# mparker97/deflate_compression

Measured on AMD Instinct MI355X. Metric: encode GB/s (uncompressed in) + compression ratio vs CPU ref, 1/2/4/8 MI355X, higher is better.
Workload: dtype u8; 1 GPU; C3: enwik8-sized enwik-style wiki text (seeded generator); bytes_per_rank=100000000, block=32768, parse=max_chain=7, lazy, store-check, deep, parallelism=blocks sharded over 1 GPU(s)

## Files before the change

deflate_compression_amd/csrc/dmx_kernels.hip:

```cpp
#include <hip/hip_runtime.h>
#include <stdint.h>
#include <stdio.h>
#include <stdlib.h>
#include <string.h>

#include "dmx_internal.h"
#include "../../include/dmx.h"

#define MAXLEN 258


__device__ __forceinline__ uint32_t dmx_hash(uint32_t tri) { return (tri * 0x9E3779B1u) >> DMX_HASH_SHIFT; }
__device__ __forceinline__ uint32_t wave_of(uint32_t tid) { return (uint32_t)__builtin_amdgcn_readfirstlane((int)(tid >> 6)); }
__device__ __forceinline__ uint32_t sort_key(uint32_t w, uint32_t p) { return (dmx_hash(w & 0xFFFFFFu) << 15) | p; }
__device__ __forceinline__ uint32_t dmx_hash4(uint32_t w) { return (w * 0x9E3779B1u) >> DMX_HASH_SHIFT; }
template <int NB>
__device__ __forceinline__ uint32_t bucket_of(uint64_t w) {
    if (NB == 3) return dmx_hash((uint32_t)w & 0xFFFFFFu);
    if (NB == 4) return dmx_hash4((uint32_t)w);
    return (uint32_t)(((w & 0xFFFFFFFFFFull) * 0x9E3779B97F4A7C15ull) >> (64 - 13));
}
template <int NB>
__device__ __forceinline__ uint32_t sort_key_h(uint64_t w, uint32_t p) { return (bucket_of<NB>(w) << 15) | p; }
template <int NB>
// ... 14 lines not shown
__device__ __forceinline__ void dist_sym(uint32_t dist, uint32_t& sym, uint32_t& eb, uint32_t& ev) {
    uint32_t x = dist - 1;
    if (x < 4) { sym = x; eb = 0; ev = 0; }
    else {
        uint32_t e = 31 - __clz(x);
        eb = e - 1;
        sym = 2 * e + ((x >> (e - 1)) & 1);
        ev = x & ((1u << eb) - 1);
    }
}

__device__ __forceinline__ uint32_t len_eb_of_sym(uint32_t s) {
    return (s >= 265 && s < 285) ? (s - 261) / 4 : 0;
}
__device__ __forceinline__ uint32_t dist_eb_of_sym(uint32_t s) { return s < 4 ? 0 : s / 2 - 1; }
__device__ __forceinline__ uint32_t fixed_len(uint32_t s) { return s < 144 ? 8 : s < 256 ? 9 : s < 280 ? 7 : 8; }

#define DMX_DPP_SHR(x, n) ((uint32_t)__builtin_amdgcn_update_dpp(0, (int)(x), 0x110 + (n), 0xF, 0xF, true))
__device__ __forceinline__ uint32_t wave_sum_u32(uint32_t v) {
    v += DMX_DPP_SHR(v, 1);
    v += DMX_DPP_SHR(v, 2);
    v += DMX_DPP_SHR(v, 4);
    v += DMX_DPP_SHR(v, 8);
    return __builtin_amdgcn_readlane(v, 15) + __builtin_amdgcn_readlane(v, 31) + __builtin_amdgcn_readlane(v, 47) +
           __builtin_amdgcn_readlane(v, 63);
}
__device__ __forceinline__ uint64_t dpp_shr64(uint64_t v, int n) {
    const uint32_t lo = (uint32_t)v, hi = (uint32_t)(v >> 32);
    uint32_t a, b;
    switch (n) {
        case 1: a = DMX_DPP_SHR(lo, 1); b = DMX_DPP_SHR(hi, 1); break;
        case 2: a = DMX_DPP_SHR(lo, 2); b = DMX_DPP_SHR(hi, 2); break;
        case 4: a = DMX_DPP_SHR(lo, 4); b = DMX_DPP_SHR(hi, 4); break;
        default: a = DMX_DPP_SHR(lo, 8); b = DMX_DPP_SHR(hi, 8); break;
    }
    return (uint64_t)a | ((uint64_t)b << 32);
}
__device__ __forceinline__ uint64_t readlane64(uint64_t v, int l) {
    return (uint64_t)(uint32_t)__builtin_amdgcn_readlane((int)(uint32_t)v, l) |
           ((uint64_t)(uint32_t)__builtin_amdgcn_readlane((int)(uint32_t)(v >> 32), l) << 32);
}
__device__ __forceinline__ uint32_t wave_claim(uint32_t* ctr) {
#ifdef DMX_CHECK_CLAIM
    if (__builtin_amdgcn_read_exec() != ~0ull) __builtin_trap();
#endif
    return atomicAdd(ctr, 1u) >> 6;
}
__device__ __forceinline__ uint64_t wave_sum_u64(uint64_t v) {
    v += dpp_shr64(v, 1);
    v += dpp_shr64(v, 2);
    v += dpp_shr64(v, 4);
    v += dpp_shr64(v, 8);
    return readlane64(v, 15) + readlane64(v, 31) + readlane64(v, 47) + readlane64(v, 63);
}


#define MT 1024
#define MW (MT / 64)
#define DMX_STAMPS 16
#define DATA_WORDS 8272

struct __attribute__((aligned(16))) MatchLDS {
    uint32_t data[DATA_WORDS];
    uint16_t sorted[DMX_BLK];
    uint16_t bstart[DMX_NBUCKET];
    uint8_t len8[DMX_BLK];
    uint32_t lit[DMX_BLK / 32];
    uint32_t tsm[DMX_BLK / 32];
    uint32_t exitp[DMX_BLK / 32];
    uint32_t hist[DMX_HIST];
    uint32_t wexit[MW];
    uint32_t wsum[MW];
    uint32_t ntok;
    uint32_t sortbad;
    unsigned long long adl_s, adl_t;
};

__device__ __forceinline__ uint64_t fsh64(uint64_t lo, uint64_t hi, uint32_t sh) {
    return sh ? ((lo >> sh) | (hi << (64 - sh))) : lo;
}
__device__ __forceinline__ uint64_t ld8(const uint32_t* W, uint32_t p) {
    const uint32_t a = p >> 2, sh = p & 3;
    const uint32_t w0 = W[a], w1 = W[a + 1], w2 = W[a + 2];
    return (uint64_t)__builtin_amdgcn_alignbyte(w1, w0, sh) | ((uint64_t)__builtin_amdgcn_alignbyte(w2, w1, sh) << 32);
}
__device__ __forceinline__ uint32_t ld4(const uint32_t* W, uint32_t p) {
    return __builtin_amdgcn_alignbyte(W[(p >> 2) + 1], W[p >> 2], p & 3);
}
template <int NB>
__device__ __forceinline__ uint64_t ldg(const uint32_t* W, uint32_t p) { return NB > 4 ? ld8(W, p) : (uint64_t)ld4(W, p); }
template <int NG>
__device__ __forceinline__ uint16_t seed_enc(uint32_t q) {
    return q != 0xFFFFu ? (uint16_t)((NG == 4 ? 0x8000u : 0u) | q) : (uint16_t)0xFFFFu;
}
__device__ __forceinline__ uint32_t seed_dec(uint32_t s) {
    return s == 0xFFFFu ? 0u : ((3u + (s >> 15)) << 15) | (s & 0x7FFFu);
}
__device__ __forceinline__ void ld12(const uint32_t* W, uint32_t p, uint32_t& x0, uint32_t& x1, uint32_t& x2) {
    const uint32_t a = p >> 2, sh = p & 3;
    const uint32_t w0 = W[a], w1 = W[a + 1], w2 = W[a + 2], w3 = W[a + 3];
    x0 = __builtin_amdgcn_alignbyte(w1, w0, sh);
    x1 = __builtin_amdgcn_alignbyte(w2, w1, sh);
    x2 = __builtin_amdgcn_alignbyte(w3, w2, sh);
}

__device__ __forceinline__ uint32_t adv_of(const MatchLDS& L, uint32_t p) {
// ... 944 lines not shown
    if (__ballot(valid && v != v0) == 0) {
        if ((threadIdx.x & 63) == first) {
            const uint32_t c = (uint32_t)__popcll(vm);
            if (pair16) atomicAdd(&T[v0 >> 1], c << (16 * (v0 & 1)));
            else atomicAdd(&T[v0], c);
        }
    } else if (valid) {
        if (pair16) atomicAdd(&T[v >> 1], 1u << (16 * (v & 1)));
        else atomicAdd(&T[v], 1u);
    }
}

template <bool RUNCHK = true>
__device__ __forceinline__ uint32_t atomic_rank(uint32_t* T, uint32_t v, bool valid, uint64_t lt) {
    if (!RUNCHK) return valid ? atomicAdd(&T[v], 1u) : 0u;
    const uint64_t vm = __ballot(valid);
    if (vm == 0) return 0;
    const uint32_t first = (uint32_t)__builtin_ctzll(vm);
    const uint32_t v0 = __builtin_amdgcn_readlane(v, (int)first);
    if (__ballot(valid && v != v0) == 0) {
        uint32_t base = 0;
        if ((threadIdx.x & 63) == first) base = atomicAdd(&T[v0], (uint32_t)__popcll(vm));
        return __builtin_amdgcn_readlane(base, (int)first) + (uint32_t)__popcll(vm & lt);
    }
    return valid ? atomicAdd(&T[v], 1u) : 0u;
}

__device__ __forceinline__ uint32_t block_excl_scan(MatchLDS& L, uint32_t v, uint32_t tid) {
    const uint32_t incl = wave_incl_scan(v);
    if ((tid & 63) == 63) L.wsum[tid >> 6] = incl;
    __syncthreads();
    uint32_t base = 0;
    for (uint32_t w = 0; w < (tid >> 6); w++) base += L.wsum[w];
    __syncthreads();
    return base + incl - v;
}

template <bool RUNCHK>
__device__ __forceinline__ uint32_t atomic_rank16(uint32_t* T, uint32_t v, bool valid, uint64_t lt, uint32_t sh) {
    if (RUNCHK) {
        const uint64_t vm = __ballot(valid);
        if (vm == 0) return 0;
        const uint32_t first = (uint32_t)__builtin_ctzll(vm);
        const uint32_t v0 = __builtin_amdgcn_readlane(v, (int)first);
        if (__ballot(valid && v != v0) == 0) {
            uint32_t base = 0;
            if ((threadIdx.x & 63) == first) base = atomicAdd(&T[v0], (uint32_t)__popcll(vm) << sh);
            return ((__builtin_amdgcn_readlane(base, (int)first) >> sh) & 0xFFFFu) + (uint32_t)__popcll(vm & lt);
        }
    }
    return (atomicAdd(&T[v], valid ? 1u << sh : 0u) >> sh) & 0xFFFFu;
}

template <bool RUNCHK, int NB>
__device__ __forceinline__ void count_sort_positions(MatchLDS& L, uint32_t bn, int32_t max_chain, uint32_t tid,
                                                     bool stamp, uint64_t* tp0) {
    const uint32_t lane = tid & 63, wave = wave_of(tid);
    const uint32_t nvalid = bn > 2 ? bn - 2 : 0;
    const bool need_starts = max_chain <= 0 || max_chain > KD;
    uint32_t* T = reinterpret_cast<uint32_t*>(L.len8);
    const uint4 z4 = make_uint4(0, 0, 0, 0);
    reinterpret_cast<uint4*>(T)[tid] = z4;
    reinterpret_cast<uint4*>(T)[tid + MT] = z4;
    uint32_t* T2 = reinterpret_cast<uint32_t*>(L.sorted);
    reinterpret_cast<uint4*>(T2)[tid] = z4;
    reinterpret_cast<uint4*>(T2)[tid + MT] = z4;
    constexpr uint32_t NR = 4;
    uint32_t* Tg = (wave >> 3) ? T2 : T;
    const uint32_t sh = ((wave >> 2) & 1) << 4;
    __syncthreads();
    const uint64_t lt = (1ull << lane) - 1ull;
    uint32_t x0l = (wave << 11) + lane, nvl = nvalid;
    uint32_t hh[16];
    asm volatile("" : "+v"(x0l), "+v"(nvl));
#pragma unroll
    for (int st = 0; st < 32; st += 2) {
        const uint32_t xa = x0l + ((uint32_t)st << 6), xb = xa + 64;
        const uint32_t ha = xa < nvl ? bucket_of<NB>(ldg<NB>(L.data, xa)) : 0u;
        const uint32_t hb = xb < nvl ? bucket_of<NB>(ldg<NB>(L.data, xb)) : 0u;
        hh[st >> 1] = ha | (hb << 16);
        if ((st & 7) == 6) __builtin_amdgcn_sched_barrier(0);
    }
    if (stamp && tid == 0) tp0[0] = __builtin_amdgcn_s_memtime();
    uint32_t rk[16];
#pragma unroll
    for (int j = 0; j < 16; j++) rk[j] = 0;
    for (uint32_t r = 0; r < NR; r++) {
        if (r == (wave & (NR - 1))) {
            asm volatile("" : "+v"(x0l), "+v"(nvl));
            if (RUNCHK) {
#pragma unroll
                for (int st = 0; st < 32; st++) {
                    const uint32_t x = x0l + ((uint32_t)st << 6);
                    const uint32_t h = (hh[st >> 1] >> (16 * (st & 1))) & 0xFFFFu;
                    const uint32_t rr = atomic_rank16<true>(Tg, h, x < nvl, lt, sh);
                    rk[st >> 1] |= rr << (16 * (st & 1));
                }
            } else {
#pragma unroll
                for (int hb = 0; hb < 32; hb += 16) {
                    uint32_t old[16];
#pragma unroll
                    for (int q = 0; q < 16; q++) {
                        const int st = hb + q;
                        const uint32_t x = x0l + ((uint32_t)st << 6);
                        const uint32_t h = (hh[st >> 1] >> (16 * (st & 1))) & 0xFFFFu;
                        old[q] = atomicAdd(&Tg[h], x < nvl ? 1u << sh : 0u);
                    }
#pragma unroll
                    for (int q = 0; q < 16; q++) {
                        const int st = hb + q;
                        rk[st >> 1] |= ((old[q] >> sh) & 0xFFFFu) << (16 * (st & 1));
                    }
                }
            }
        }
        __syncthreads();
    }
    if (stamp && tid == 0) tp0[1] = __builtin_amdgcn_s_memtime();
    {
        const uint4 a = reinterpret_cast<const uint4*>(T)[2 * tid], c = reinterpret_cast<const uint4*>(T)[2 * tid + 1];
        uint32_t w[8] = {a.x, a.y, a.z, a.w, c.x, c.y, c.z, c.w}, pre[8], s = 0;
        const uint4 a2 = reinterpret_cast<const uint4*>(T2)[2 * tid], c2 = reinterpret_cast<const uint4*>(T2)[2 * tid + 1];
        uint32_t w2[8] = {a2.x, a2.y, a2.z, a2.w, c2.x, c2.y, c2.z, c2.w};
#pragma unroll
        for (int j = 0; j < 8; j++) {
            pre[j] = s;
            s += (w[j] & 0xFFFFu) + (w[j] >> 16);
            s += (w2[j] & 0xFFFFu) + (w2[j] >> 16);
        }
        const uint32_t base = block_excl_scan(L, s, tid);
#pragma unroll
        for (int j = 0; j < 8; j++) {
            const uint32_t st0 = base + pre[j];
            pre[j] = st0;
            const uint32_t s1 = st0 + (w[j] & 0xFFFFu), s2 = s1 + (w[j] >> 16);
            w[j] = st0 | (s1 << 16);
            w2[j] = s2 | ((s2 + (w2[j] & 0xFFFFu)) << 16);
        }
        reinterpret_cast<uint4*>(T)[2 * tid] = make_uint4(w[0], w[1], w[2], w[3]);
        reinterpret_cast<uint4*>(T)[2 * tid + 1] = make_uint4(w[4], w[5], w[6], w[7]);
        reinterpret_cast<uint4*>(T2)[2 * tid] = make_uint4(w2[0], w2[1], w2[2], w2[3]);
        reinterpret_cast<uint4*>(T2)[2 * tid + 1] = make_uint4(w2[4], w2[5], w2[6], w2[7]);
        if (need_starts)
            reinterpret_cast<uint4*>(L.bstart)[tid] = make_uint4(pre[0] | (pre[1] << 16), pre[2] | (pre[3] << 16),
                                                                 pre[4] | (pre[5] << 16), pre[6] | (pre[7] << 16));
    }
    __syncthreads();
    asm volatile("" : "+v"(x0l), "+v"(nvl));
#pragma unroll
    for (int st = 0; st < 32; st++) {
        const uint32_t h = (hh[st >> 1] >> (16 * (st & 1))) & 0xFFFFu;
        const uint32_t rr = (rk[st >> 1] >> (16 * (st & 1))) & 0xFFFFu;
        const uint32_t dst = ((Tg[h] >> sh) & 0xFFFFu) + rr;
        rk[st >> 1] = (rk[st >> 1] & (0xFFFF0000u >> (16 * (st & 1)))) | ((dst & 0xFFFFu) << (16 * (st & 1)));
        if ((st & 7) == 7) __builtin_amdgcn_sched_barrier(0);
    }
    __syncthreads();
#pragma unroll
    for (int st = 0; st < 32; st++) {
        const uint32_t x = x0l + ((uint32_t)st << 6);
        if (x < nvl) L.sorted[(rk[st >> 1] >> (16 * (st & 1))) & 0xFFFFu] = (uint16_t)x;
    }
    __syncthreads();
    if (stamp && tid == 0) tp0[2] = __builtin_amdgcn_s_memtime();
}

template <bool EXACT, bool RUNCHK = true, int NB = 3>
__device__ __forceinline__ void sort_positions(MatchLDS& L, uint32_t bn, int32_t max_chain, uint32_t tid, bool stamp,
                                               uint64_t* tp0) {
    if constexpr (!EXACT) {
        count_sort_positions<RUNCHK, NB>(L, bn, max_chain, tid, stamp, tp0);
        return;
    }
    const uint32_t lane = tid & 63, wave = wave_of(tid);
    const uint32_t nvalid = bn > 2 ? bn - 2 : 0;
    const bool need_starts = max_chain <= 0 || max_chain > KD;
    uint32_t* C = L.tsm;
    uint32_t* C2 = L.lit;
    uint8_t* D2 = reinterpret_cast<uint8_t*>(L.bstart);
    unsigned long long* G = reinterpret_cast<unsigned long long*>(L.len8 + DMX_BLK / 2);
    unsigned long long* Gw = G + (wave << 7);
    for (uint32_t k = tid; k < 2 * (DMX_BLK / 32); k += MT) C[k] = 0;
    for (uint32_t k = tid; k < DMX_BLK / 32; k += MT) C2[k] = 0;
    for (uint32_t k = tid; k < 16 * 128; k += MT) G[k] = 0;
    __syncthreads();
    if (stamp && tid == 0) tp0[0] = __builtin_amdgcn_s_memtime();
    const uint64_t lt = (1ull << lane) - 1ull;
    const uint32_t x0 = (wave << 11) + lane;
    uint32_t x0l = x0, nvl = nvalid;
    uint32_t hh[16];
    asm volatile("" : "+v"(x0l), "+v"(nvl));
#pragma unroll
    for (int st = 0; st < 32; st += 2) {
        const uint32_t xa = x0l + ((uint32_t)st << 6), xb = xa + 64;
        const uint32_t ha = xa < nvl ? bucket_of<NB>(ldg<NB>(L.data, xa)) : 0u;
        const uint32_t hb = xb < nvl ? bucket_of<NB>(ldg<NB>(L.data, xb)) : 0u;
        hh[st >> 1] = ha | (hb << 16);
        if ((st & 7) == 6) __builtin_amdgcn_sched_barrier(0);
    }
    asm volatile("" : "+v"(x0l), "+v"(nvl));
#pragma unroll
    for (int st = 0; st < 32; st++) {
        const uint32_t x = x0l + ((uint32_t)st << 6);
        const uint32_t h = (hh[st >> 1] >> (16 * (st & 1))) & 0xFFFFu;
        count_add<RUNCHK>(C + (wave << 7), h & 127u, x < nvl, false);
    }
    __syncthreads();
    {
        const uint32_t o0 = tid * 2, o1 = o0 + 1;
        const uint32_t i0 = ((o0 & 15) << 7) + (o0 >> 4), i1 = ((o1 & 15) << 7) + (o1 >> 4);
        const uint32_t v0 = C[i0], v1 = C[i1];
        const uint32_t ex = block_excl_scan(L, v0 + v1, tid);
        C[i0] = ex;
        C[i1] = ex + v0;
    }
    __syncthreads();
    asm volatile("" : "+v"(x0l), "+v"(nvl));
#pragma unroll
    for (int st = 0; st < 32; st++) {
        const uint32_t x = x0l + ((uint32_t)st << 6);
        const bool valid = x < nvl;
        const uint32_t h = (hh[st >> 1] >> (16 * (st & 1))) & 0xFFFFu;
        const uint32_t dg = h & 127u;
        uint32_t dst = 0;
        if (EXACT) {
            const uint32_t c = valid ? C[(wave << 7) + dg] : 0u;
// ... 14 lines not shown
    if (stamp && tid == 0) tp0[1] = __builtin_amdgcn_s_memtime();
    uint32_t pk[16], dk[8];
    asm volatile("" : "+v"(x0l), "+v"(nvl));
#pragma unroll
    for (int st = 0; st < 32; st += 2) {
        const uint32_t xa = x0l + ((uint32_t)st << 6), xb = xa + 64;
        const uint32_t pa = xa < nvl ? (uint32_t)L.sorted[xa] : 0u;
        const uint32_t pb = xb < nvl ? (uint32_t)L.sorted[xb] : 0u;
        const uint32_t da = xa < nvl ? (uint32_t)D2[xa] : 0u;
        const uint32_t db = xb < nvl ? (uint32_t)D2[xb] : 0u;
        pk[st >> 1] = pa | (pb << 16);
        if ((st & 3) == 0) dk[st >> 2] = da | (db << 8);
        else dk[st >> 2] |= (da << 16) | (db << 24);
        if ((st & 7) == 6) __builtin_amdgcn_sched_barrier(0);
    }
    {
        const uint32_t i0 = ((tid & 15) << 6) + (tid >> 4);
        const uint32_t v0 = C2[i0];
        const uint32_t ex = block_excl_scan(L, v0, tid);
        C2[i0] = ex;
    }
    __syncthreads();
    asm volatile("" : "+v"(x0l), "+v"(nvl));
#pragma unroll
    for (int st = 0; st < 32; st++) {
        const uint32_t x = x0l + ((uint32_t)st << 6);
        const bool valid = x < nvl;
        const uint32_t p = (pk[st >> 1] >> (16 * (st & 1))) & 0xFFFFu;
        const uint32_t dg = (dk[st >> 2] >> (8 * (st & 3))) & 0xFFu;
        if (EXACT) {
            const uint32_t c = valid ? C2[(wave << 6) + dg] : 0u;
            const uint64_t eq = group_of(Gw, dg, valid);
            if (valid) {
                L.sorted[c + (uint32_t)__popcll(eq & lt)] = (uint16_t)p;
                if ((eq >> lane) == 1ull) C2[(wave << 6) + dg] = c + (uint32_t)__popcll(eq);
            }
        } else {
            const uint32_t dst = atomic_rank<RUNCHK>(&C2[wave << 6], dg, valid, lt);
            if (valid) L.sorted[dst] = (uint16_t)p;
        }
        __builtin_amdgcn_sched_barrier(0);
    }
    __syncthreads();
    for (uint32_t k = tid; k < DMX_BLK / 32; k += MT) L.lit[k] = 0;
    if (need_starts) {
        for (uint32_t k = tid; k < nvalid; k += MT) {
            const uint32_t h = bucket_of<NB>(ldg<NB>(L.data, L.sorted[k]));
            const uint32_t hp = k ? bucket_of<NB>(ldg<NB>(L.data, L.sorted[k - 1])) : 0xFFFFFFFFu;
            if (h != hp) L.bstart[h] = (uint16_t)k;
        }
    }
    __syncthreads();
    if (stamp && tid == 0) tp0[2] = __builtin_amdgcn_s_memtime();
}


template <int NG>
__device__ __forceinline__ uint32_t gram_pass(MatchLDS& L, uint32_t nv, uint32_t tid, uint16_t* __restrict__ seeds,
                                              uint32_t& ndefer, uint64_t& tsweep) {
    constexpr uint32_t PW = 9;
    constexpr uint32_t GM = NG == 3 ? 0xFFFFFFu : 0xFFFFFFFFu;
    const uint32_t lane = tid & 63;
    uint32_t* UL = L.tsm;
    uint32_t bad = 0;
    if (tid == 0) { L.ntok = 0; L.wsum[0] = 0; L.wsum[1] = 0; }
    __syncthreads();
    uint32_t cnx = wave_claim(&L.wsum[0]);
    for (;;) {
        const uint32_t kb = (uint32_t)__builtin_amdgcn_readfirstlane((int)cnx) << 6;
        if (kb >= nv) break;
        cnx = wave_claim(&L.wsum[0]);
        const uint32_t k = kb + lane;
        const bool act = k < nv;
        const uint32_t i = act ? (uint32_t)L.sorted[k] : 0u, w = act ? ld4(L.data, i) : 0u;
        const uint32_t t = w & GM, hb = bucket_of<NG>(t);
        uint32_t hi = 0xFFFFu, hw = 0;
        if (lane < PW && kb >= lane + 1) { hi = L.sorted[kb - 1 - lane]; hw = ld4(L.data, hi); }
        uint32_t ip = i, wp = w, q = 0xFFFFu;
        bool open = act && k > 0;
        for (uint32_t st = 1; st <= PW; st++) {
            if (st > 1 && !__ballot(open)) break;
            ip = wshr(ip, __builtin_amdgcn_readlane(hi, (int)st - 1));
            wp = wshr(wp, __builtin_amdgcn_readlane(hw, (int)st - 1));
            if (st == 1 && open && sort_key_h<NG>(wp, ip) > sort_key_h<NG>(w, i)) bad = 1;
            if (open && k >= st) {
                if ((wp & GM) == t) { q = ip; open = false; }
                else if (bucket_of<NG>(wp & GM) != hb) open = false;
            } else {
                open = false;
            }
        }
        if (open && k > PW) {
            const uint32_t u = atomicAdd(&L.ntok, 1u);
            if (u < 2 * (DMX_BLK / 32)) {
                UL[u] = ((k - PW) << 16) | k;
            } else {
                for (uint32_t j = k - PW; j > 0; j--) {
                    const uint32_t c = L.sorted[j - 1], wc = ld4(L.data, c) & GM;
                    if (wc == t) { q = c; break; }
                    if (bucket_of<NG>(wc) != hb) break;
                }
            }
        }
        if (act && (NG == 3 || (q != 0xFFFFu && i + NG <= nv + 2))) seeds[i] = seed_enc<NG>(q);
    }
    __syncthreads();
// ... 487 lines not shown
            for (int k = 0; k < 8; k++) red[k][wave] = ones[k];
        }
        const uint32_t c4 = (uint32_t)d[0] * 0x01010101u;
        const bool u0 = w[0] == c4 && w[1] == c4 && w[2] == c4 && w[3] == c4;
        const bool uni4k = __syncthreads_and(u0) != 0;
        if (tid == 0) {
            bool ok = true;
            for (int k = 0; k < 8; k++) {
                int64_t o = 0;
#pragma unroll
                for (int w2 = 0; w2 < SCT / 64; w2++) o += (int64_t)red[k][w2];
                const int64_t dv = 2 * o - (int64_t)SC_PLANE;
                ok = ok && 8 * (dv < 0 ? -dv : dv) <= (int64_t)SC_PLANE;
            }
            pass_s = ok ? 1u : 0u;
            if (!ok) info[b].prestored = 0;
        }
        __syncthreads();
        if (!pass_s) {
            if (!uni_ok || !uni4k) return 0u;
            bool u = true;
            for (uint32_t p = (tid + SCT) << 4; p < bn; p += SCT << 4) {
                uint32_t x[5];
                sc_load(d, p, bn, aligned16, x);
                const uint32_t nb = bn - p < 16 ? bn - p : 16;
#pragma unroll
                for (int q = 0; q < 4; q++) {
                    const uint32_t m = 4 * q + 4 <= (int)nb ? 0xFFFFFFFFu : (4 * q >= nb ? 0u : (1u << (8 * (nb - 4 * q))) - 1u);
                    u = u && ((x[q] ^ c4) & m) == 0;
                }
            }
            if (!__syncthreads_and(u)) return 0u;
            uint32_t* H = bm;
            for (uint32_t k = tid; k < DMX_HIST; k += SCT) H[k] = 0;
            __syncthreads();
            const uint32_t c = c4 & 0xFFu;
            const uint32_t nt = uniform_parse(bn, c, tok_g + (uint64_t)b * DMX_BLK, H, tid, SCT);
            if (tid == 0) {
                const uint64_t S = (uint64_t)c * bn, T = (uint64_t)c * ((uint64_t)bn * (bn - 1) / 2);
                info[b].ntok = nt;
                info[b].n = bn;
                info[b].adl_s = S;
                info[b].adl_w = (uint64_t)bn * S - T;
                info[b].prestored = 2u | ((bn == sw && b >= 1 && b + 2 <= nblk) ? 4u | (c << 8) : 0u);
            }
            __syncthreads();
            for (uint32_t k = tid; k < DMX_HIST; k += SCT) hist_g[(uint64_t)b * DMX_HIST + k] = H[k];
            return 2u | ((bn == sw && b >= 1 && b + 2 <= nblk) ? 4u | (c << 8) : 0u);
        }
    }
    uint64_t s = 0, t = 0;
    auto chunk1 = [&](uint32_t p, const uint32_t* w) {
        uint32_t ts = 0, tt = 0;
#pragma unroll
        for (int q = 0; q < 4; q++) {
            ts = __builtin_amdgcn_sad_u8(w[q], 0u, ts);
            tt = __builtin_amdgcn_udot4(w[q], 0x03020100u + 0x04040404u * q, tt, false);
        }
        s += ts;
        t += (uint64_t)p * ts + tt;
    };
    if (full) {
        if (!SPEC) load_full();
#pragma unroll
        for (int i = 0; i < 8; i++) {
            const uint32_t w[4] = {v[i].x, v[i].y, v[i].z, v[i].w};
            chunk1((tid + i * SCT) << 4, w);
        }

    } else {
        for (uint32_t p = tid << 4; p < bn; p += SCT << 4) {
            uint32_t w[5];
            sc_load(d, p, bn, aligned16, w);
            chunk1(p, w);
        }
    }
    s = wave_sum_u64(s);
    t = wave_sum_u64(t);
    if (lane == 0) {
        red[8][wave] = s;
        red[9][wave] = t;
    }
    for (uint32_t k = tid; k < (1u << 12) / 4; k += SCT) reinterpret_cast<uint4*>(bm)[k] = make_uint4(0, 0, 0, 0);
    hist[tid] = 0;
    __syncthreads();
    uint32_t qn = 0;
    const uint32_t smask = bn >= 32768 ? 7u : bn >= 16384 ? 3u : bn >= 8192 ? 1u : 0u;
    auto chunk2 = [&](uint32_t p, const uint32_t* w) {
#pragma unroll
        for (int j = 0; j < 16; j++) {
            const uint32_t lo = w[j >> 2], hi = w[(j >> 2) + 1];
            const uint32_t g4 = (j & 3) ? __builtin_amdgcn_alignbyte(hi, lo, (uint32_t)(j & 3)) : lo;
            if (((uint32_t)j & smask) == 0 && p + j < bn) atomicAdd(&hist[(lo >> (8 * (j & 3))) & 0xFFu], 1u);
            const uint32_t x = g4 * 0x9E3779B1u;
            if (p + j + 4 <= bn && !(x & (7u << 11))) {
                qn++;
                atomicOr(&bm[x >> 20], 1u << ((x >> 15) & 31));
            }
        }
    };
    if (full) {
#ifndef DMX_K0_NOPASS2
#pragma unroll
        for (int i = 0; i < 8; i++) {
            const uint32_t w[5] = {v[i].x, v[i].y, v[i].z, v[i].w, next4(i)};
            chunk2((tid + i * SCT) << 4, w);
        }
#endif
    } else {
        for (uint32_t p = tid << 4; p < bn; p += SCT << 4) {
            uint32_t w[5];
// ... 343 lines not shown
        const uint8_t* d = in + (uint64_t)b * sw;
#ifdef DMX_K0_NOREST
        if (b < nblk && wl_skip(b, wl[WL_M], nblk))
#else
        if (b < nblk && wl_skip(b, wl[WL_M], nblk) && !(sw == SCT * 16 * 8 && (reinterpret_cast<uintptr_t>(d) & 15) == 0))
#endif
            stored_rest(d, sw, spec_stored_bit(b, sw, flags), lane & 15, 16, out32);
    }
    if (!dedupe) return;
    for (uint32_t i = 0; i < 4; i++) {
        const uint32_t b = b0 + i;
        if (b >= nblk || !(wl_codes(wl, cap)[b] & 8u)) continue;
        const uint32_t r = wl_dup(wl, cap)[b];
        uint64_t Ob = info[b].off_bits, Or = info[r].off_bits, Lb = info[b].len_bits;
        if (flags & DMX_F_BGZF) {
            Ob -= 144;
            Or -= 144;
            Lb = 144 + ((Lb + 7) & ~7ull) + 64;
        }
        const uint64_t gw0 = Ob >> 5;
        const uint32_t nwords = (uint32_t)(((Ob & 31) + Lb + 31) >> 5);
        for (uint32_t k = lane; k < nwords; k += 64) {
            const uint64_t lo = 32 * (gw0 + k), hi = lo + 32;
            const uint64_t a = lo > Ob ? lo : Ob, e = hi < Ob + Lb ? hi : Ob + Lb;
            const uint64_t q = a - Ob + Or;
            const uint64_t qw = q >> 5;
            const uint32_t sh = (uint32_t)(q & 31);
            const uint64_t src = (uint64_t)out32[qw] | ((uint64_t)out32[qw + 1] << 32);
            const uint32_t nb = (uint32_t)(e - a);
            const uint64_t bits = (src >> sh) & ((1ull << nb) - 1ull);
            const uint32_t v = (uint32_t)(bits << (a - lo));
            if (nb == 32) out32[gw0 + k] = v;
            else atomicOr(&out32[gw0 + k], v);
        }
    }
}

__device__ __forceinline__ bool dbg_stop(uint32_t mflags, uint32_t phase, dmx_blkinfo* info, uint32_t* hist_g,
                                         uint32_t b, uint32_t bn, uint32_t tid) {
    if (((mflags >> 8) & 3u) != phase) return false;
    for (uint32_t k = tid; k < DMX_HIST; k += MT) hist_g[(uint64_t)b * DMX_HIST + k] = 0;
    if (tid == 0) {
        info[b].ntok = 0;
        info[b].n = bn;
        info[b].adl_s = 0;
        info[b].adl_w = 0;
        info[b].prestored = 0;
    }
    return true;
}

__device__ __forceinline__ int32_t block_chain(MatchLDS& L, uint32_t bn, int32_t max_chain, uint32_t mflags,
                                               uint32_t tid) {
    const int32_t dk = (mflags >> 16) & 0xFFu ? (int32_t)((mflags >> 16) & 0xFFu) : (int32_t)DMX_DEEP_CHAIN;
    if (!(mflags & 8u) || max_chain <= 0 || max_chain >= dk) return max_chain;
    const uint32_t nvalid = bn > 2 ? bn - 2 : 0;
    uint32_t* SB = L.hist;
#pragma unroll
    for (uint32_t j = 0; j < 4; j++) {
        const uint32_t p = (((tid >> 8) + 4 * j) << 11) | (tid & 255u);
        if (p < nvalid) {
            const uint32_t h = dmx_hash(ld4(L.data, p) & 0xFFFFFFu);
            atomicOr(&SB[h >> 5], 1u << (h & 31));
        }
    }
    __syncthreads();
    if (tid < DMX_NBUCKET / 32) {
        const uint32_t c = wave_sum_u32((uint32_t)__popc(SB[tid]));
        SB[tid] = 0;
        if ((tid & 63) == 0) atomicAdd(&L.ntok, c);
    }
    __syncthreads();
    uint32_t ns = 0;
    for (uint32_t s = 0; s < 16; s++) {
        const uint32_t lo = s << 11;
        ns += nvalid > lo ? min(nvalid - lo, 256u) : 0u;
    }
    return 4 * L.ntok < ns ? dk : max_chain;
}

#ifndef DMX_NBX
#define DMX_NBX 4
#endif
__device__ __forceinline__ uint4 stage16(const uint8_t* __restrict__ d, uint32_t p, uint32_t bn, bool aligned16) {
    if (aligned16 && p + 16 <= bn) return *reinterpret_cast<const uint4*>(d + p);
    uint32_t w[4] = {0, 0, 0, 0};
    for (uint32_t j = 0; j < 16; j++)
        if (p + j < bn) w[j >> 2] |= (uint32_t)d[p + j] << (8 * (j & 3));
    return make_uint4(w[0], w[1], w[2], w[3]);
}
template <bool DICT, int NBX, bool LOOP = false>
__device__ __forceinline__ void match_block(const uint32_t b, const uint8_t* __restrict__ in, uint64_t n, uint32_t sw,
                                            int32_t max_chain, uint32_t mflags, uint16_t* __restrict__ dist_g,
                                            const uint16_t* __restrict__ chs, uint32_t* __restrict__ tok_g,
                                            uint32_t* __restrict__ hist_g,
                                            dmx_blkinfo* __restrict__ info, uint64_t* __restrict__ dbg,
                                            uint32_t* __restrict__ nfallback) {
    __shared__ MatchLDS L;
    __shared__ uint64_t st_search, st_iters, st_w1, st_w23, st_def, tp0[3], st_rounds, st_p3a, st_h4[3], st_lz, st_w1w;
    uint32_t tid = threadIdx.x;
    if (LOOP) asm volatile("" : "+v"(tid));
    const uint32_t lane = tid & 63, wave = wave_of(tid);
    const uint64_t off = (uint64_t)b * sw;
    const uint32_t bn = (uint32_t)((n - off) < sw ? (n - off) : sw);
    const uint8_t* d = in + off;
    const bool aligned16 = ((reinterpret_cast<uintptr_t>(d) & 15) == 0);
    const uint32_t pst = info[b].prestored;
    constexpr bool early = !LOOP;
    uint4 v0 = make_uint4(0, 0, 0, 0), v1 = v0;
    if (early) {
        v0 = stage16(d, tid << 4, bn, aligned16);
        v1 = stage16(d, (tid + MT) << 4, bn, aligned16);
    }
    if ((mflags & 4u) && pst) return;
    uint16_t* pg = dist_g + (uint64_t)b * DMX_BLK;
    uint8_t* D8 = reinterpret_cast<uint8_t*>(L.data);

    const uint64_t tbeg = dbg ? __builtin_amdgcn_s_memtime() : 0;
    if (tid == 0) { L.adl_s = 0; L.adl_t = 0; L.sortbad = (mflags & 2u) ? 1u : 0u; L.ntok = 0; }
    if (dbg && tid == 0) { st_search = 0; st_iters = 0; st_def = 0; st_p3a = 0; }
    for (uint32_t k = tid; k < DMX_HIST; k += MT) L.hist[k] = 0;
    for (uint32_t k = tid; k < DMX_BLK / 32; k += MT) L.lit[k] = 0;
    uint32_t runny = 0;
    bool uni = true;
    uint32_t cb = 0x100u;
    for (uint32_t k = tid; k < DATA_WORDS / 4; k += MT) {
        const uint32_t p = k << 4;
        uint4 v;
        if (early && k < 2 * MT) v = k < MT ? v0 : v1;
        else v = stage16(d, p, bn, aligned16);
        *reinterpret_cast<uint4*>(&L.data[k << 2]) = v;
        const bool rep = v.x == v.y && v.y == v.z && v.z == v.w && v.x == (v.x & 0xFFu) * 0x01010101u;
        runny += (p < bn && rep) ? 1u : 0u;
        if (p + 16 <= bn) {
            uni = uni && rep && (cb == 0x100u || cb == (v.x & 0xFFu));
            cb = v.x & 0xFFu;
        } else if (p < bn) {
            const uint32_t w4[4] = {v.x, v.y, v.z, v.w};
            const uint32_t c0 = cb == 0x100u ? (v.x & 0xFFu) : cb;
            for (uint32_t j = 0; j < bn - p; j++) uni = uni && ((w4[j >> 2] >> (8 * (j & 3))) & 0xFFu) == c0;
            cb = c0;
        }
    }
    runny = wave_sum_u32(runny);
    if (lane == 0) L.wexit[wave] = runny;
    const uint32_t* hbk = DICT ? tok_g + (uint64_t)b * DMX_BLK : nullptr;
    int32_t kb = max_chain;
    if (DICT) {
        const uint32_t nv = bn > 2 ? bn - 2 : 0;
        const uint16_t* Sg = chs + (uint64_t)(b + 1) * DMX_BLK;
        for (uint32_t k = tid; k < (nv + 7) / 8; k += MT)
            reinterpret_cast<uint4*>(L.sorted)[k] = reinterpret_cast<const uint4*>(Sg)[k];
        for (uint32_t k = tid; k < DMX_BLK / 32; k += MT) L.lit[k] = 0;
        __syncthreads();
        kb = block_chain(L, bn, max_chain, mflags, tid);
        if (kb <= 0 || kb > KD) {
            for (uint32_t k = tid; k < nv; k += MT) {
                const uint32_t h = dmx_hash(ld4(L.data, L.sorted[k]) & 0xFFFFFFu);
                const uint32_t hp = k ? dmx_hash(ld4(L.data, L.sorted[k - 1]) & 0xFFFFFFu) : 0xFFFFFFFFu;
                if (h != hp) L.bstart[h] = (uint16_t)k;
            }
        }
        __syncthreads();
    } else {
        if (__syncthreads_and(uni) && __syncthreads_and(cb == 0x100u || cb == (uint32_t)D8[0])) {
            const uint32_t c = D8[0];
            const uint32_t nt = uniform_parse(bn, c, tok_g + (uint64_t)b * DMX_BLK, L.hist, tid, MT);
            if (tid == 0) {
                const uint64_t S = (uint64_t)c * bn, T = (uint64_t)c * ((uint64_t)bn * (bn - 1) / 2);
                info[b].ntok = nt;
                info[b].n = bn;
                info[b].adl_s = S;
                info[b].adl_w = (uint64_t)bn * S - T;
                info[b].prestored = 0;
            }
            __syncthreads();
            for (uint32_t k = tid; k < DMX_HIST; k += MT) hist_g[(uint64_t)b * DMX_HIST + k] = L.hist[k];
            return;
        }
        uint32_t nrun0 = 0;
#pragma unroll
        for (int w = 0; w < MW; w++) nrun0 += L.wexit[w];
        kb = block_chain(L, bn, max_chain, mflags, tid);
        const int32_t mc0 = (NBX > 3 && !DICT) ? 1 : kb;
        if (nrun0 * 4 >= ((bn + 15) >> 4)) sort_positions<false, true>(L, bn, mc0, tid, dbg != nullptr, tp0);
        else sort_positions<false, false>(L, bn, mc0, tid, dbg != nullptr, tp0);
    }

    if (dbg_stop(mflags, 1, info, hist_g, b, bn, tid)) return;
    {
        uint64_t s = 0, t = 0;
        const uint32_t lo = tid << 5;
        const uint4 v0 = *reinterpret_cast<const uint4*>(&L.data[lo >> 2]);
        const uint4 v1 = *reinterpret_cast<const uint4*>(&L.data[(lo >> 2) + 4]);
        const uint32_t w[8] = {v0.x, v0.y, v0.z, v0.w, v1.x, v1.y, v1.z, v1.w};
#pragma unroll
        for (uint32_t j = 0; j < 32; j++) {
            const uint32_t c = (w[j >> 2] >> (8 * (j & 3))) & 0xFFu;
            s += c;
            t += (uint64_t)(lo + j) * c;
        }
        s = wave_sum_u64(s);
        t = wave_sum_u64(t);
        if (lane == 0) { atomicAdd(&L.adl_s, (unsigned long long)s); atomicAdd(&L.adl_t, (unsigned long long)t); }
    }

    constexpr bool h4 = NBX > 3 && !DICT;
    uint16_t* seeds = reinterpret_cast<uint16_t*>(tok_g + (uint64_t)b * DMX_BLK);
    if constexpr (h4) {
        const uint32_t nv = bn > 2 ? bn - 2 : 0;
        const uint32_t hook = L.sortbad;
        uint32_t npass = 0, ndefer = 0;
        uint64_t tsw = 0;
        for (uint32_t pass = 0;; pass++) {
            npass++;
            if (!__syncthreads_or(gram_pass<3>(L, nv, tid, seeds, ndefer, tsw)) || pass) break;
            if (tid == 0) atomicAdd(nfallback, 1u);
            sort_positions<true>(L, bn, 1, tid, false, tp0);
        }
        if constexpr (NBX > 4) {
            for (uint32_t pass = 0;; pass++) {
                npass++;
                if (hook || pass) sort_positions<true, true, 4>(L, bn, max_chain, tid, false, tp0);
                else sort_positions<false, true, 4>(L, bn, max_chain, tid, false, tp0);
                if (!__syncthreads_or(gram_pass<4>(L, nv, tid, seeds, ndefer, tsw)) || pass || hook) break;
                if (tid == 0) atomicAdd(nfallback, 1u);
            }
        }
        if (dbg && tid == 0) st_h4[0] = (__builtin_amdgcn_s_memtime() - tbeg) | ((uint64_t)npass << 48);
        if (dbg && tid == 0) st_h4[2] = tsw - tbeg;
        uint32_t nr4 = 0;
#pragma unroll
        for (int w = 0; w < MW; w++) nr4 += L.wexit[w];
        if (hook) sort_positions<true, true, NBX>(L, bn, max_chain, tid, false, tp0);
        else if (nr4 * 4 >= ((bn + 15) >> 4)) sort_positions<false, true, NBX>(L, bn, max_chain, tid, false, tp0);
        else sort_positions<false, false, NBX>(L, bn, max_chain, tid, false, tp0);
        if (dbg && tid == 0) st_h4[1] = (__builtin_amdgcn_s_memtime() - tbeg) | ((uint64_t)min(ndefer, 65535u) << 48);
    }

    const uint64_t t0 = dbg ? __builtin_amdgcn_s_memtime() : 0;
    uint64_t tdef = 0;
    for (uint32_t attempt = 0;; attempt++) {
        uint32_t nrun = 0;
#pragma unroll
        for (int w = 0; w < MW; w++) nrun += L.wexit[w];
        const bool runs = kb > 0 && kb <= KE && nrun * 4 >= ((bn + 15) >> 4);
        if (kb > 0 && kb <= KE) {
            uint32_t z = 0;
            asm volatile("" : "+v"(z));
            reinterpret_cast<uint4*>(nib_words(L))[tid] = make_uint4(z, z, z, z);
        }
        if (tid == 0) L.ntok = 0;
        __syncthreads();
        const uint32_t its = runs ? search_positions<DICT, true>(L, bn, kb, pg, tid, dbg != nullptr, tdef, hbk)
                             : h4 ? search_positions<DICT, false, (h4 ? NBX : 3)>(L, bn, kb, pg, tid, dbg != nullptr, tdef, hbk, seeds)
                                  : search_positions<DICT, false>(L, bn, kb, pg, tid, dbg != nullptr, tdef, hbk);
        if (dbg && lane == 0 && attempt == 0) {
            atomicAdd((unsigned long long*)&st_iters, (unsigned long long)its);
// ... 8 lines not shown
    }
    const uint64_t t1 = dbg ? __builtin_amdgcn_s_memtime() : 0;
    if (dbg_stop(mflags, 2, info, hist_g, b, bn, tid)) return;

    if (mflags & 1u) {
        const uint32_t lw = L.lit[tid];
        const uint32_t nb0 = (tid + 1 < DMX_BLK / 32) ? (L.lit[tid + 1] & 1u) : 1u;
        const uint32_t* l32 = reinterpret_cast<const uint32_t*>(L.len8);
        uint32_t lv[9];
#pragma unroll
        for (int j = 0; j < 8; j++) lv[j] = l32[tid * 8 + j];
        lv[8] = (tid + 1 < DMX_BLK / 32) ? l32[tid * 8 + 8] : 0u;
        const uint32_t litn = (lw >> 1) | (nb0 << 31);
        uint32_t longer = 0;
#pragma unroll
        for (int bb = 0; bb < 32; bb++) {
            const uint32_t cur = (lv[bb >> 2] >> (8 * (bb & 3))) & 0xFFu;
            const uint32_t nxt = (lv[(bb + 1) >> 2] >> (8 * ((bb + 1) & 3))) & 0xFFu;
            longer |= (nxt > cur ? 1u : 0u) << bb;
        }
        __syncthreads();
        L.lit[tid] = lw | (~lw & ~litn & longer);
        __syncthreads();
    }
    if (dbg && tid == 0) st_lz = __builtin_amdgcn_s_memtime() - t1;

    {
        const uint32_t lo = tid << 5, lw = L.lit[tid];
        uint32_t m = 0, p = lo;
        while (p < lo + 32 && p < bn) {
            const uint32_t sh = p - lo;
            const uint32_t run = min(ffbl_hw(~(lw >> sh)), min(lo + 32u, bn) - p);
            if (run) {
                m |= (run >= 32u ? ~0u : ((1u << run) - 1u)) << sh;
                p += run;
                continue;
            }
            m |= 1u << sh;
            p += (uint32_t)L.len8[p] + 3u;
        }
        L.tsm[tid] = m;
        L.exitp[tid] = p;
    }
    {
        __syncthreads();
        if (dbg && tid == 0) st_w1w = __builtin_amdgcn_s_memtime() - t1;
        const uint32_t nvalid = bn > 2 ? bn - 2 : 0;
        uint4 dv[4], pv[4];
        if (kb > 0 && kb <= KE) {
            const uint32_t* NW = nib_words(L);
#pragma unroll
            for (int j = 0; j < 4; j++) {
                const uint32_t c = tid + (uint32_t)j * MT;
                const bool in = c * 8 < nvalid;
                pv[j] = in ? reinterpret_cast<const uint4*>(L.sorted)[c] : make_uint4(0, 0, 0, 0);
                const uint32_t nw = in ? NW[c] : 0u;
                const uint32_t pw[4] = {pv[j].x, pv[j].y, pv[j].z, pv[j].w};
                uint32_t dw[4] = {0, 0, 0, 0};
#pragma unroll
                for (int e = 0; e < 8; e++) {
                    const uint32_t jj = (nw >> (4 * e)) & 15u, kk = c * 8 + (uint32_t)e;
                    uint32_t dist = 0;
                    if (jj == NIB_HIST) dist = DICT ? (hbk[kk] & 0xFFFFu) : 0u;
                    else if (jj) dist = ((pw[e >> 1] >> (16 * (e & 1))) & 0xFFFFu) - (uint32_t)L.sorted[kk - jj];
                    dw[e >> 1] |= dist << (16 * (e & 1));
                }
                dv[j] = make_uint4(dw[0], dw[1], dw[2], dw[3]);
            }
        } else {
#pragma unroll
            for (int j = 0; j < 4; j++) {
                const uint32_t c = tid + (uint32_t)j * MT;
                const bool in = c * 8 < nvalid;
                dv[j] = in ? reinterpret_cast<const uint4*>(pg)[c] : make_uint4(0, 0, 0, 0);
                pv[j] = in ? reinterpret_cast<const uint4*>(L.sorted)[c] : make_uint4(0, 0, 0, 0);
            }
        }
        __syncthreads();
#pragma unroll
        for (int j = 0; j < 4; j++) {
            const uint32_t dw[4] = {dv[j].x, dv[j].y, dv[j].z, dv[j].w}, pw[4] = {pv[j].x, pv[j].y, pv[j].z, pv[j].w};
#pragma unroll
            for (int e = 0; e < 8; e++) {
                const uint32_t kk = (tid + (uint32_t)j * MT) * 8 + (uint32_t)e;
                const uint32_t d16 = (dw[e >> 1] >> (16 * (e & 1))) & 0xFFFFu;
                if (kk < nvalid && d16 != 0) L.sorted[(pw[e >> 1] >> (16 * (e & 1))) & 0xFFFFu] = (uint16_t)d16;
            }
        }
    }
    if (dbg && tid == 0) st_w1 = __builtin_amdgcn_s_memtime() - t1;
    bool conv = false, serial = false;
    if (tid == 0) L.ntok = 0;
    {
        uint32_t entry = tid << 5;
        uint32_t r = 0;
        for (; r < JR; r++) {
            if (r == 3) {
                const uint32_t pc = wave_sum_u32((uint32_t)__popc(L.tsm[tid]));
                if (lane == 0) atomicAdd(&L.ntok, pc);
                __syncthreads();
                if (L.ntok <= WALK_SERIAL) { serial = true; break; }
            }
            const uint32_t e = tid == 0 ? 0u : L.exitp[tid - 1];
            __syncthreads();
            const bool ch = (tid << 5) < bn && e != entry;
            if (ch) {
                uint32_t nm;
                bool mg;
                const uint32_t x = resolve_word(L, tid << 5, e, bn, L.tsm[tid], L.lit[tid], L.exitp[tid], nm, mg);
                L.tsm[tid] = nm;
                L.exitp[tid] = x;
                entry = e;
            }
            if (!__syncthreads_or(ch)) { conv = true; break; }
        }
        if (dbg && tid == 0) st_rounds = r;
    }
    if (serial) {
        {
            conv = true;
            L.tsm[tid] = 0;
            __syncthreads();
            if (tid == 0) {
                uint32_t p = 0, wi = 0, cw = 0;
                while (p < bn) {
                    if ((p >> 5) != wi) { L.tsm[wi] = cw; cw = 0; wi = p >> 5; }
                    cw |= 1u << (p & 31);
                    p += adv_of(L, p);
                }
                L.tsm[wi] = cw;
            }
            __syncthreads();
        }
    }
    if (!conv) {
        {
            uint32_t myw = L.tsm[tid];
            const uint32_t myx = L.exitp[tid], myl = L.lit[tid];
            uint32_t e = wave << 11;
// ... 2208 lines not shown
```

Measured before the change: 90.67 GB/s.

## Fuse Adler checksum and deep-chain statistic into staging and counting sort

```diff
diff --git a/deflate_compression_amd/csrc/dmx_kernels.hip b/deflate_compression_amd/csrc/dmx_kernels.hip
--- a/deflate_compression_amd/csrc/dmx_kernels.hip
+++ b/deflate_compression_amd/csrc/dmx_kernels.hip
@@ -90,6 +90,25 @@
     v += dpp_shr64(v, 4);
     v += dpp_shr64(v, 8);
     return readlane64(v, 15) + readlane64(v, 31) + readlane64(v, 47) + readlane64(v, 63);
+}
+__device__ __forceinline__ uint64_t wave_sum_u32_wide(uint32_t v) {
+    v += DMX_DPP_SHR(v, 1);
+    v += DMX_DPP_SHR(v, 2);
+    v += DMX_DPP_SHR(v, 4);
+    v += DMX_DPP_SHR(v, 8);
+    return (uint64_t)(uint32_t)__builtin_amdgcn_readlane(v, 15) + (uint32_t)__builtin_amdgcn_readlane(v, 31) +
+           (uint32_t)__builtin_amdgcn_readlane(v, 47) + (uint32_t)__builtin_amdgcn_readlane(v, 63);
+}
+typedef uint16_t dmx_u16x2 __attribute__((ext_vector_type(2)));
+__device__ __forceinline__ uint32_t pk_sub_u16(uint32_t a, uint32_t b) {
+    return __builtin_bit_cast(uint32_t, __builtin_bit_cast(dmx_u16x2, a) - __builtin_bit_cast(dmx_u16x2, b));
+}
+__device__ __forceinline__ void adler16(const uint32_t* w, uint32_t& ts, uint32_t& tt) {
+#pragma unroll
+    for (int q = 0; q < 4; q++) {
+        ts = __builtin_amdgcn_sad_u8(w[q], 0u, ts);
+        tt = __builtin_amdgcn_udot4(w[q], 0x03020100u + 0x04040404u * q, tt, false);
+    }
 }
 
 
@@ -1140,9 +1159,22 @@
     return (atomicAdd(&T[v], valid ? 1u << sh : 0u) >> sh) & 0xFFFFu;
 }
 
-template <bool RUNCHK, int NB>
-__device__ __forceinline__ void count_sort_positions(MatchLDS& L, uint32_t bn, int32_t max_chain, uint32_t tid,
-                                                     bool stamp, uint64_t* tp0) {
+__device__ __forceinline__ int32_t deep_chain_of(uint32_t mflags) {
+    return (mflags >> 16) & 0xFFu ? (int32_t)((mflags >> 16) & 0xFFu) : (int32_t)DMX_DEEP_CHAIN;
+}
+__device__ __forceinline__ uint32_t deep_samples(uint32_t nvalid) {
+    uint32_t ns = 0;
+    for (uint32_t s = 0; s < 16; s++) {
+        const uint32_t lo = s << 11;
+        ns += nvalid > lo ? min(nvalid - lo, 256u) : 0u;
+    }
+    return ns;
+}
+
+template <bool RUNCHK, int NB, bool DEEP>
+__device__ __forceinline__ int32_t count_sort_positions(MatchLDS& L, uint32_t bn, int32_t max_chain, uint32_t tid,
+                                                        bool stamp, uint64_t* tp0, int32_t deep_dk) {
+    static_assert(!DEEP || NB == 3, "the depth statistic hashes trigrams");
     const uint32_t lane = tid & 63, wave = wave_of(tid);
     const uint32_t nvalid = bn > 2 ? bn - 2 : 0;
     const bool need_starts = max_chain <= 0 || max_chain > KD;
@@ -1169,11 +1201,25 @@
         hh[st >> 1] = ha | (hb << 16);
         if ((st & 7) == 6) __builtin_amdgcn_sched_barrier(0);
     }
+    const bool deep = DEEP && deep_dk > 0;
+    if (deep) {
+#pragma unroll
+        for (int st = 0; st < 4; st++) {
+            const uint32_t h = (hh[st >> 1] >> (16 * (st & 1))) & 0xFFFFu;
+            if (x0l + ((uint32_t)st << 6) < nvl) atomicOr(&L.hist[h >> 5], 1u << (h & 31));
+        }
+    }
     if (stamp && tid == 0) tp0[0] = __builtin_amdgcn_s_memtime();
     uint32_t rk[16];
 #pragma unroll
     for (int j = 0; j < 16; j++) rk[j] = 0;
     for (uint32_t r = 0; r < NR; r++) {
+        if (deep && r == 1 && wave < 8 && !(wave & 1)) {
+            const uint32_t k = (wave << 5) + lane;
+            const uint32_t c = wave_sum_u32((uint32_t)__popc(L.hist[k]));
+            L.hist[k] = 0;
+            if (lane == 0) atomicAdd(&L.ntok, c);
+        }
         if (r == (wave & (NR - 1))) {
             asm volatile("" : "+v"(x0l), "+v"(nvl));
             if (RUNCHK) {
@@ -1206,6 +1252,7 @@
         __syncthreads();
     }
     if (stamp && tid == 0) tp0[1] = __builtin_amdgcn_s_memtime();
+    const int32_t kb = deep && 4 * L.ntok < deep_samples(nvalid) ? deep_dk : max_chain;
     {
         const uint4 a = reinterpret_cast<const uint4*>(T)[2 * tid], c = reinterpret_cast<const uint4*>(T)[2 * tid + 1];
         uint32_t w[8] = {a.x, a.y, a.z, a.w, c.x, c.y, c.z, c.w}, pre[8], s = 0;
@@ -1252,15 +1299,14 @@
     }
     __syncthreads();
     if (stamp && tid == 0) tp0[2] = __builtin_amdgcn_s_memtime();
-}
-
-template <bool EXACT, bool RUNCHK = true, int NB = 3>
-__device__ __forceinline__ void sort_positions(MatchLDS& L, uint32_t bn, int32_t max_chain, uint32_t tid, bool stamp,
-                                               uint64_t* tp0) {
-    if constexpr (!EXACT) {
-        count_sort_positions<RUNCHK, NB>(L, bn, max_chain, tid, stamp, tp0);
-        return;
-    }
+    return kb;
+}
+
+template <bool EXACT, bool RUNCHK = true, int NB = 3, bool DEEP = false>
+__device__ __forceinline__ int32_t sort_positions(MatchLDS& L, uint32_t bn, int32_t max_chain, uint32_t tid, bool stamp,
+                                                  uint64_t* tp0, int32_t deep_dk = 0) {
+    static_assert(!(EXACT && DEEP), "only the counting sort takes the depth statistic along");
+    if constexpr (!EXACT) return count_sort_positions<RUNCHK, NB, DEEP>(L, bn, max_chain, tid, stamp, tp0, deep_dk);
     const uint32_t lane = tid & 63, wave = wave_of(tid);
     const uint32_t nvalid = bn > 2 ? bn - 2 : 0;
     const bool need_starts = max_chain <= 0 || max_chain > KD;
@@ -1381,6 +1427,7 @@
     }
     __syncthreads();
     if (stamp && tid == 0) tp0[2] = __builtin_amdgcn_s_memtime();
+    return max_chain;
 }
 
 
@@ -1974,11 +2021,7 @@
     uint64_t s = 0, t = 0;
     auto chunk1 = [&](uint32_t p, const uint32_t* w) {
         uint32_t ts = 0, tt = 0;
-#pragma unroll
-        for (int q = 0; q < 4; q++) {
-            ts = __builtin_amdgcn_sad_u8(w[q], 0u, ts);
-            tt = __builtin_amdgcn_udot4(w[q], 0x03020100u + 0x04040404u * q, tt, false);
-        }
+        adler16(w, ts, tt);
         s += ts;
         t += (uint64_t)p * ts + tt;
     };
@@ -2428,7 +2471,7 @@
 
 __device__ __forceinline__ int32_t block_chain(MatchLDS& L, uint32_t bn, int32_t max_chain, uint32_t mflags,
                                                uint32_t tid) {
-    const int32_t dk = (mflags >> 16) & 0xFFu ? (int32_t)((mflags >> 16) & 0xFFu) : (int32_t)DMX_DEEP_CHAIN;
+    const int32_t dk = deep_chain_of(mflags);
     if (!(mflags & 8u) || max_chain <= 0 || max_chain >= dk) return max_chain;
     const uint32_t nvalid = bn > 2 ? bn - 2 : 0;
     uint32_t* SB = L.hist;
@@ -2447,12 +2490,7 @@
         if ((tid & 63) == 0) atomicAdd(&L.ntok, c);
     }
     __syncthreads();
-    uint32_t ns = 0;
-    for (uint32_t s = 0; s < 16; s++) {
-        const uint32_t lo = s << 11;
-        ns += nvalid > lo ? min(nvalid - lo, 256u) : 0u;
-    }
-    return 4 * L.ntok < ns ? dk : max_chain;
+    return 4 * L.ntok < deep_samples(nvalid) ? dk : max_chain;
 }
 
 #ifndef DMX_NBX
@@ -2500,12 +2538,20 @@
     uint32_t runny = 0;
     bool uni = true;
     uint32_t cb = 0x100u;
+    uint32_t as = 0, at = 0;
     for (uint32_t k = tid; k < DATA_WORDS / 4; k += MT) {
         const uint32_t p = k << 4;
         uint4 v;
         if (early && k < 2 * MT) v = k < MT ? v0 : v1;
         else v = stage16(d, p, bn, aligned16);
         *reinterpret_cast<uint4*>(&L.data[k << 2]) = v;
+        {
+            const uint32_t w[4] = {v.x, v.y, v.z, v.w};
+            uint32_t ts = 0, tt = 0;
+            adler16(w, ts, tt);
+            as += ts;
+            at += p * ts + tt;
+        }
         const bool rep = v.x == v.y && v.y == v.z && v.z == v.w && v.x == (v.x & 0xFFu) * 0x01010101u;
         runny += (p < bn && rep) ? 1u : 0u;
         if (p + 16 <= bn) {
@@ -2520,6 +2566,8 @@
     }
     runny = wave_sum_u32(runny);
     if (lane == 0) L.wexit[wave] = runny;
+    const uint32_t adl_ws = wave_sum_u32(as);
+    const uint64_t adl_wt = wave_sum_u32_wide(at);
     const uint32_t* hbk = DICT ? tok_g + (uint64_t)b * DMX_BLK : nullptr;
     int32_t kb = max_chain;
     if (DICT) {
@@ -2529,6 +2577,7 @@
             reinterpret_cast<uint4*>(L.sorted)[k] = reinterpret_cast<const uint4*>(Sg)[k];
         for (uint32_t k = tid; k < DMX_BLK / 32; k += MT) L.lit[k] = 0;
         __syncthreads();
+        if (lane == 0) { atomicAdd(&L.adl_s, (unsigned long long)adl_ws); atomicAdd(&L.adl_t, (unsigned long long)adl_wt); }
         kb = block_chain(L, bn, max_chain, mflags, tid);
         if (kb <= 0 || kb > KD) {
             for (uint32_t k = tid; k < nv; k += MT) {
@@ -2554,32 +2603,22 @@
             for (uint32_t k = tid; k < DMX_HIST; k += MT) hist_g[(uint64_t)b * DMX_HIST + k] = L.hist[k];
             return;
         }
+        if (lane == 0) { atomicAdd(&L.adl_s, (unsigned long long)adl_ws); atomicAdd(&L.adl_t, (unsigned long long)adl_wt); }
         uint32_t nrun0 = 0;
 #pragma unroll
         for (int w = 0; w < MW; w++) nrun0 += L.wexit[w];
-        kb = block_chain(L, bn, max_chain, mflags, tid);
+        const int32_t dk = deep_chain_of(mflags);
+        const bool insort = NBX == 3 && (mflags & 8u) && max_chain > 0 && max_chain < dk && dk <= KD;
+        const int32_t sort_dk = insort ? dk : 0;
+        if (!insort) kb = block_chain(L, bn, max_chain, mflags, tid);
         const int32_t mc0 = (NBX > 3 && !DICT) ? 1 : kb;
-        if (nrun0 * 4 >= ((bn + 15) >> 4)) sort_positions<false, true>(L, bn, mc0, tid, dbg != nullptr, tp0);
-        else sort_positions<false, false>(L, bn, mc0, tid, dbg != nullptr, tp0);
+        const int32_t ks = nrun0 * 4 >= ((bn + 15) >> 4)
+                               ? sort_positions<false, true, 3, NBX == 3>(L, bn, mc0, tid, dbg != nullptr, tp0, sort_dk)
+                               : sort_positions<false, false, 3, NBX == 3>(L, bn, mc0, tid, dbg != nullptr, tp0, sort_dk);
+        if (insort) kb = ks;
     }
 
     if (dbg_stop(mflags, 1, info, hist_g, b, bn, tid)) return;
-    {
-        uint64_t s = 0, t = 0;
-        const uint32_t lo = tid << 5;
-        const uint4 v0 = *reinterpret_cast<const uint4*>(&L.data[lo >> 2]);
-        const uint4 v1 = *reinterpret_cast<const uint4*>(&L.data[(lo >> 2) + 4]);
-        const uint32_t w[8] = {v0.x, v0.y, v0.z, v0.w, v1.x, v1.y, v1.z, v1.w};
-#pragma unroll
-        for (uint32_t j = 0; j < 32; j++) {
-            const uint32_t c = (w[j >> 2] >> (8 * (j & 3))) & 0xFFu;
-            s += c;
-            t += (uint64_t)(lo + j) * c;
-        }
-        s = wave_sum_u64(s);
-        t = wave_sum_u64(t);
-        if (lane == 0) { atomicAdd(&L.adl_s, (unsigned long long)s); atomicAdd(&L.adl_t, (unsigned long long)t); }
-    }
 
     constexpr bool h4 = NBX > 3 && !DICT;
     uint16_t* seeds = reinterpret_cast<uint16_t*>(tok_g + (uint64_t)b * DMX_BLK);
@@ -2694,18 +2733,27 @@
 #pragma unroll
             for (int j = 0; j < 4; j++) {
                 const uint32_t c = tid + (uint32_t)j * MT;
-                const bool in = c * 8 < nvalid;
-                pv[j] = in ? reinterpret_cast<const uint4*>(L.sorted)[c] : make_uint4(0, 0, 0, 0);
-                const uint32_t nw = in ? NW[c] : 0u;
+                pv[j] = reinterpret_cast<const uint4*>(L.sorted)[c];
+                const uint32_t nw = NW[c];
                 const uint32_t pw[4] = {pv[j].x, pv[j].y, pv[j].z, pv[j].w};
-                uint32_t dw[4] = {0, 0, 0, 0};
+                uint32_t j2[2] = {(nw << 1) & 0x1E1E1E1Eu, (nw >> 3) & 0x1E1E1E1Eu};
+                asm("" : "+v"(j2[0]), "+v"(j2[1]));
+                const uint8_t* S8 = reinterpret_cast<const uint8_t*>(L.sorted);
+                uint32_t cs[8];
 #pragma unroll
                 for (int e = 0; e < 8; e++) {
-                    const uint32_t jj = (nw >> (4 * e)) & 15u, kk = c * 8 + (uint32_t)e;
-                    uint32_t dist = 0;
-                    if (jj == NIB_HIST) dist = DICT ? (hbk[kk] & 0xFFFFu) : 0u;
-                    else if (jj) dist = ((pw[e >> 1] >> (16 * (e & 1))) & 0xFFFFu) - (uint32_t)L.sorted[kk - jj];
-                    dw[e >> 1] |= dist << (16 * (e & 1));
+                    uint32_t jj = (j2[e & 1] >> (8 * (e >> 1))) & 0xFFu;
+                    if (DICT) jj = jj == 2u * NIB_HIST ? 0u : jj;
+                    cs[e] = (uint32_t)*reinterpret_cast<const uint16_t*>(S8 + (c * 16 + 2 * (uint32_t)e - jj));
+                }
+                uint32_t dw[4];
+#pragma unroll
+                for (int q = 0; q < 4; q++) dw[q] = pk_sub_u16(pw[q], cs[2 * q] | (cs[2 * q + 1] << 16));
+                if (DICT) {
+#pragma unroll
+                    for (int e = 0; e < 8; e++)
+                        if (((nw >> (4 * e)) & 15u) == NIB_HIST)
+                            dw[e >> 1] |= (hbk[c * 8 + (uint32_t)e] & 0xFFFFu) << (16 * (e & 1));
                 }
                 dv[j] = make_uint4(dw[0], dw[1], dw[2], dw[3]);
             }
@@ -2716,17 +2764,26 @@
                 const bool in = c * 8 < nvalid;
                 dv[j] = in ? reinterpret_cast<const uint4*>(pg)[c] : make_uint4(0, 0, 0, 0);
                 pv[j] = in ? reinterpret_cast<const uint4*>(L.sorted)[c] : make_uint4(0, 0, 0, 0);
+                if (c == nvalid >> 3) {
+                    const uint32_t cut = nvalid & 7u;
+                    uint32_t dw[4] = {dv[j].x, dv[j].y, dv[j].z, dv[j].w};
+#pragma unroll
+                    for (uint32_t q = 0; q < 4; q++) dw[q] &= cut >= 2 * q + 2 ? ~0u : cut == 2 * q + 1 ? 0xFFFFu : 0u;
+                    dv[j] = make_uint4(dw[0], dw[1], dw[2], dw[3]);
+                }
             }
         }
         __syncthreads();
 #pragma unroll
         for (int j = 0; j < 4; j++) {
-            const uint32_t dw[4] = {dv[j].x, dv[j].y, dv[j].z, dv[j].w}, pw[4] = {pv[j].x, pv[j].y, pv[j].z, pv[j].w};
+            const uint32_t dw[4] = {dv[j].x, dv[j].y, dv[j].z, dv[j].w};
+            uint32_t p2[4] = {pv[j].x << 1, pv[j].y << 1, pv[j].z << 1, pv[j].w << 1};
+            asm("" : "+v"(p2[0]), "+v"(p2[1]), "+v"(p2[2]), "+v"(p2[3]));
 #pragma unroll
             for (int e = 0; e < 8; e++) {
-                const uint32_t kk = (tid + (uint32_t)j * MT) * 8 + (uint32_t)e;
                 const uint32_t d16 = (dw[e >> 1] >> (16 * (e & 1))) & 0xFFFFu;
-                if (kk < nvalid && d16 != 0) L.sorted[(pw[e >> 1] >> (16 * (e & 1))) & 0xFFFFu] = (uint16_t)d16;
+                const uint32_t o2 = (e & 1) ? p2[e >> 1] >> 16 : p2[e >> 1] & 0xFFFFu;
+                if (d16 != 0) *reinterpret_cast<uint16_t*>(reinterpret_cast<uint8_t*>(L.sorted) + o2) = (uint16_t)d16;
             }
         }
     }
```

Result: faster. 94.27 GB/s, median of 6 (+4.0%).
